# ruanyyyyyyy/point-cloud-process

Hardware: AMD Instinct MI355X
Metric: correspondence-pairs/sec + ms/ICP-iter, 120k-pt KITTI pair (higher is better)
Workload: dtype f64; 1 GPU; point-to-point ICP iteration, 120000 x 120000 KITTI-shaped synthetic scan pair per GPU (BASELINE configs[1]); exact 1-NN via grid; nn=grid, pairs_per_gpu=1, points_src=120000, points_tgt=120000

## Files before the change

include/pcr.h:

```cpp
#ifndef PCR_H
#define PCR_H

#include <stdint.h>

#ifdef __cplusplus
extern "C" {
#endif

#define PCR_API __attribute__((visibility("default")))

enum {
    PCR_OK = 0,
    PCR_E_TOO_FEW_ASSOC = 1,
    PCR_E_INVALID = -1,
    PCR_E_EMPTY = -2,
    PCR_E_NOMEM = -3,
    PCR_E_HIP = -4,
    PCR_E_NO_DEVICE = -5,
    PCR_E_UNSUPPORTED = -6,
    PCR_E_TOO_MANY_ITERS = -7,
    PCR_E_SINGULAR = -8
};

typedef struct pcr_ctx pcr_ctx;
typedef struct pcr_cloud pcr_cloud;
typedef struct pcr_index pcr_index;

PCR_API const char* pcr_strerror(int status);
PCR_API const char* pcr_last_error(const pcr_ctx* ctx);
PCR_API const char* pcr_version(void);

PCR_API int pcr_ctx_create(int device, pcr_ctx** out);
PCR_API int pcr_ctx_destroy(pcr_ctx* ctx);
PCR_API int pcr_ctx_sync(pcr_ctx* ctx);
PCR_API int pcr_ctx_device_info(pcr_ctx* ctx, char* name256, int* cu_count, int64_t* hbm_bytes);

PCR_API int pcr_cloud_upload_f32(pcr_ctx* ctx, const float* xyz, int64_t n, int64_t stride_floats, pcr_cloud** out);
PCR_API int pcr_cloud_upload_f64(pcr_ctx* ctx, const double* xyz, int64_t n, int64_t stride_doubles, pcr_cloud** out);
PCR_API int pcr_cloud_download_f64(pcr_ctx* ctx, const pcr_cloud* cloud, double* xyz_out );
PCR_API int64_t pcr_cloud_size(const pcr_cloud* cloud);
PCR_API int pcr_cloud_reordered(const pcr_cloud* cloud);
PCR_API int pcr_cloud_free(pcr_ctx* ctx, pcr_cloud* cloud);
PCR_API int pcr_cloud_prepare(pcr_ctx* ctx, pcr_cloud* cloud, const pcr_index* index);
PCR_API int pcr_cloud_transform(pcr_ctx* ctx, pcr_cloud* cloud, const double T[16]);

enum { PCR_INDEX_GRID = 0, PCR_INDEX_BRUTE = 1 };
PCR_API int pcr_index_build(pcr_ctx* ctx, const pcr_cloud* target, int kind, double cell, pcr_index** out);
PCR_API int pcr_index_free(pcr_ctx* ctx, pcr_index* index);
PCR_API int pcr_index_kind(const pcr_index* index);
PCR_API double pcr_index_cell(const pcr_index* index);
PCR_API int64_t pcr_index_size(const pcr_index* index);

PCR_API int pcr_nn1(pcr_ctx* ctx, const pcr_index* index, const pcr_cloud* queries, const double* T ,
                    double max_d2, int32_t* idx_out, double* d2_out);

PCR_API int pcr_knn(pcr_ctx* ctx, const pcr_index* index, const double* queries_xyz, int64_t q, int k,
                    int32_t* idx_out, double* dist_out);
PCR_API int pcr_radius(pcr_ctx* ctx, const pcr_index* index, const double* queries_xyz, int64_t q, double radius,
                       int64_t* counts_out, const int64_t* offsets, int32_t* idx_out, double* dist_out);

PCR_API int pcr_radius_small(pcr_ctx* ctx, const pcr_index* index, const double* queries_xyz, int q, double radius, int64_t cap,
                             int64_t* counts_out, int32_t* idx_out, double* dist_out);

enum { PCR_ICP_COMPAT_MAIN = 0,
       PCR_ICP_TOTAL = 1         };
enum { PCR_RMETRIC_FROBENIUS = 0, PCR_RMETRIC_GEODESIC = 1 };
#define PCR_ICP_MAX_LOG 256

typedef struct pcr_icp_params {
    int32_t max_iter;
    double r_thres;
    double t_thres;
    double max_d2;
    int32_t mode;
// ... 328 lines not shown
```

point-cloud-process_amd/_lib.py:

```python
from __future__ import annotations

import ctypes as C
import os
import sys

import numpy as np

_HERE = os.path.dirname(os.path.abspath(__file__))
LIB_PATH = os.environ.get("PCR_LIB_PATH") or os.path.join(_HERE, "libpcr.so")

PCR_OK = 0
PCR_E_TOO_FEW_ASSOC = 1
PCR_E_INVALID = -1
PCR_E_EMPTY = -2
PCR_E_NOMEM = -3
PCR_E_HIP = -4
PCR_E_NO_DEVICE = -5
PCR_E_UNSUPPORTED = -6
PCR_E_TOO_MANY_ITERS = -7
PCR_E_SINGULAR = -8

PCR_INDEX_GRID = 0
PCR_INDEX_BRUTE = 1
PCR_ICP_COMPAT_MAIN = 0
# ... 230 lines not shown
        ("kmeans_converged", C.c_int32),
        ("n_empty", C.c_int32),
        ("n_edges", C.c_int64),
        ("eigenvalues", C.c_double * 8),
        ("residuals", C.c_double * 8),
        ("next_eigenvalue", C.c_double),
        ("inertia", C.c_double),
        ("graph_ms", C.c_double),
        ("solver_ms", C.c_double),
        ("kmeans_ms", C.c_double),
        ("reserved", C.c_double * 4),
    ]


_vp = C.c_void_p
_dp = C.POINTER(C.c_double)
_fp = C.POINTER(C.c_float)
_ip = C.POINTER(C.c_int32)
_lp = C.POINTER(C.c_int64)

SIGNATURES = {
    "pcr_strerror": (C.c_char_p, [C.c_int]),
    "pcr_last_error": (C.c_char_p, [_vp]),
    "pcr_version": (C.c_char_p, []),
    "pcr_ctx_create": (C.c_int, [C.c_int, C.POINTER(_vp)]),
    "pcr_ctx_destroy": (C.c_int, [_vp]),
    "pcr_ctx_sync": (C.c_int, [_vp]),
    "pcr_ctx_device_info": (C.c_int, [_vp, C.c_char_p, C.POINTER(C.c_int), _lp]),
    "pcr_cloud_upload_f32": (C.c_int, [_vp, _fp, C.c_int64, C.c_int64, C.POINTER(_vp)]),
    "pcr_cloud_upload_f64": (C.c_int, [_vp, _dp, C.c_int64, C.c_int64, C.POINTER(_vp)]),
    "pcr_cloud_download_f64": (C.c_int, [_vp, _vp, _dp]),
    "pcr_cloud_size": (C.c_int64, [_vp]),
    "pcr_cloud_reordered": (C.c_int, [_vp]),
    "pcr_cloud_free": (C.c_int, [_vp, _vp]),
    "pcr_cloud_transform": (C.c_int, [_vp, _vp, _dp]),
    "pcr_cloud_prepare": (C.c_int, [_vp, _vp, _vp]),
    "pcr_index_build": (C.c_int, [_vp, _vp, C.c_int, C.c_double, C.POINTER(_vp)]),
    "pcr_index_free": (C.c_int, [_vp, _vp]),
    "pcr_index_kind": (C.c_int, [_vp]),
    "pcr_index_cell": (C.c_double, [_vp]),
    "pcr_index_size": (C.c_int64, [_vp]),
    "pcr_nn1": (C.c_int, [_vp, _vp, _vp, _dp, C.c_double, _ip, _dp]),
    "pcr_knn": (C.c_int, [_vp, _vp, _dp, C.c_int64, C.c_int, _ip, _dp]),
    "pcr_radius": (C.c_int, [_vp, _vp, _dp, C.c_int64, C.c_double, _lp, _lp, _ip, _dp]),
    "pcr_radius_small": (C.c_int, [_vp, _vp, _dp, C.c_int, C.c_double, C.c_int64, _lp, _ip, _dp]),
    "pcr_icp_default_params": (None, [C.POINTER(IcpParams)]),
    "pcr_icp": (C.c_int, [_vp, _vp, _vp, C.POINTER(IcpParams), _dp, C.POINTER(IcpResult)]),
    "pcr_index_set_normals": (C.c_int, [_vp, _vp, _dp]),
    "pcr_index_has_normals": (C.c_int, [_vp]),
    "pcr_icp_plane_default_params": (None, [C.POINTER(IcpPlaneParams)]),
    "pcr_icp_point2plane": (C.c_int, [_vp, _vp, _vp, C.POINTER(IcpPlaneParams), _dp, C.POINTER(IcpPlaneResult)]),
    "pcr_point2plane_moments": (C.c_int, [_vp, _vp, _vp, _dp, C.c_double, _dp]),
    "pcr_point2plane_solve": (C.c_int, [_dp, _dp, _dp, _dp]),
    "pcr_icp_batch": (C.c_int, [C.POINTER(_vp), C.c_int, C.POINTER(Pair), C.c_int64, C.POINTER(IcpParams), C.POINTER(IcpResult), _ip]),
    "pcr_global_default_params": (C.c_int, [C.c_double, C.POINTER(GlobalParams)]),
    "pcr_register_pairs": (C.c_int, [C.POINTER(_vp), C.c_int, C.POINTER(CloudRef), C.c_int64, C.POINTER(PairRef), C.c_int64, C.POINTER(GlobalParams),
                                     C.POINTER(IcpParams), C.POINTER(IcpResult), _ip, _dp]),
    "pcr_match_pairs_fused": (C.c_int, [_vp, _dp, _lp, C.c_int64, _ip, C.c_int64, C.c_int, _ip, _dp, _ip, _dp, _ip, _ip]),
    "pcr_icp_moments": (C.c_int, [_vp, _vp, _vp, _dp, C.c_double, _dp, _dp, _dp]),
    "pcr_procrustes": (C.c_int, [_dp, _dp, C.c_int64, _dp, _dp, _dp]),
    "pcr_homo2tq": (C.c_int, [_dp, _dp]),
    "pcr_voxel_keys": (C.c_int, [_vp, _dp, C.c_int64, C.c_double, _dp, _dp]),
    "pcr_voxel_filter": (C.c_int, [_vp, _dp, C.c_int64, C.c_double, C.c_int, C.c_uint64, _dp, _lp]),
    "pcr_voxel_filter_cloud": (C.c_int, [_vp, _vp, C.c_double, C.c_int, C.c_uint64, C.POINTER(_vp)]),
    "pcr_iss": (C.c_int, [_vp, _vp, C.c_double, C.c_double, C.c_double, C.c_double, C.c_int, _dp, _ip, _ip, C.POINTER(C.c_int)]),
    "pcr_pca": (C.c_int, [_vp, _vp, _dp, _dp, _dp]),
# ... 127 lines not shown
```

point-cloud-process_amd/csrc/pcr_core.hip:

```cpp
#include <algorithm>
#include <cmath>
#include <cstdio>
#include <cstring>
#include <cstdlib>
#include <chrono>
#include <thread>
#include <atomic>
#include <memory>
#include <utility>
#include <vector>
#include "pcr_internal.h"

extern "C" {

const char* pcr_version(void) { return "pcr 0.1 (gfx950, f64)"; }

const char* pcr_strerror(int s) {
    switch (s) {
        case PCR_OK: return "ok";
        case PCR_E_TOO_FEW_ASSOC: return "ICP failed, cannot find enough associations!";
        case PCR_E_INVALID: return "invalid argument";
        case PCR_E_EMPTY: return "empty point cloud";
        case PCR_E_NOMEM: return "out of memory";
        case PCR_E_HIP: return "HIP runtime error";
// ... 543 lines not shown
    hipLaunchKernelGGL(expand_cloud_kernel<S>, dim3(grid), dim3(block), 0, ctx->stream, d_src, (long long)n, (long long)stride, c->d,
                       (unsigned long long*)pcr_counter(ctx, PCR_CW_BOX), h_box_dev);
    PCR_HIP(ctx, hipGetLastError());
    PCR_HIP(ctx, pcr_sync(ctx->stream));
    {
        double lo[3], hi[3];
        bool finite = true;
        for (int k = 0; k < 3; ++k) {
            hi[k] = ordered_value(h_box[k]);
            lo[k] = -ordered_value(h_box[3 + k]);
            finite = finite && std::isfinite(lo[k]) && std::isfinite(hi[k]);
        }
        if (finite) {
            c->has_bbox = true;
            for (int k = 0; k < 3; ++k) { c->lo[k] = lo[k] == 0.0 ? 0.0 : lo[k]; c->hi[k] = hi[k]; }
        }
    }
    if (timing) {
        const auto t_2 = std::chrono::steady_clock::now();
        fprintf(stderr, "upload n=%lld stride=%lld: host copy + box %.1f us, expand kernel + sync %.1f us\n", (long long)n, (long long)stride,
                std::chrono::duration_cast<std::chrono::nanoseconds>(t_1 - t_0).count() / 1e3, std::chrono::duration_cast<std::chrono::nanoseconds>(t_2 - t_1).count() / 1e3);
    }
    *out = c.release();
    return PCR_OK;
}

__global__ void cloud_rows_kernel(const pcr_pt* __restrict__ in, long long n, pcr_pt* __restrict__ out) {
    long long i = (long long)blockIdx.x * blockDim.x + threadIdx.x;
    if (i >= n) return;
    const pcr_pt p = in[i];
    out[p.id] = p;
}

int pcr_cloud_rows(pcr_ctx* ctx, const pcr_cloud* c, pcr_pt* d_out) {
    hipLaunchKernelGGL(cloud_rows_kernel, dim3((unsigned)((c->n + 255) / 256)), dim3(256), 0, ctx->stream, (const pcr_pt*)c->d, (long long)c->n, d_out);
    PCR_HIP(ctx, hipGetLastError());
    return PCR_OK;
}

__global__ void __launch_bounds__(256)
cloud_gather_rows_kernel(const pcr_pt* __restrict__ pts, long long n, const long long* __restrict__ rows, const long long* __restrict__ slot, int m,
                         double* __restrict__ out) {
    const long long i = (long long)blockIdx.x * blockDim.x + threadIdx.x;
    if (i >= n) return;
    const pcr_pt r = pts[i];
    int lo = 0, hi = m;
    while (lo < hi) {
        const int mid = (lo + hi) >> 1;
        if (rows[mid] < r.id) lo = mid + 1; else hi = mid;
    }
    for (; lo < m && rows[lo] == r.id; ++lo) {
        const long long s = slot ? slot[lo] : lo;
        out[3 * s] = r.x; out[3 * s + 1] = r.y; out[3 * s + 2] = r.z;
    }
}

int pcr_cloud_gather_rows(pcr_ctx* ctx, const pcr_cloud* c, const long long* d_rows_sorted, const long long* d_slot, int64_t m, double* d_xyz_out) {
    hipLaunchKernelGGL(cloud_gather_rows_kernel, dim3((unsigned)((c->n + 255) / 256)), dim3(256), 0, ctx->stream, (const pcr_pt*)c->d, (long long)c->n,
                       d_rows_sorted, d_slot, (int)m, d_xyz_out);
    PCR_HIP(ctx, hipGetLastError());
    return PCR_OK;
}

constexpr int64_t PCR_DOWNLOAD_MAX_ROWS = 4096;

extern "C" {
// ... 17 lines not shown
    int grid = (int)((c->n + block - 1) / block);
    hipLaunchKernelGGL(pack_xyz_kernel, dim3(grid), dim3(block), 0, ctx->stream, (const pcr_pt*)c->d, (long long)c->n, d_tmp);
    PCR_HIP(ctx, hipGetLastError());
    PCR_HIP(ctx, hipMemcpyAsync(out, d_tmp, sizeof(double) * 3 * c->n, hipMemcpyDeviceToHost, ctx->stream));
    PCR_HIP(ctx, pcr_sync(ctx->stream));
    return PCR_OK;
}

int pcr_cloud_download_rows(pcr_ctx* ctx, const pcr_cloud* cloud, const int64_t* rows, int64_t m, double* xyz_out) try {
    if (!ctx || !cloud || !rows || !xyz_out || m < 0 || m > PCR_DOWNLOAD_MAX_ROWS) return PCR_E_INVALID;
    if (m == 0) return PCR_OK;
    const int64_t n = cloud->n;
    std::vector<std::pair<long long, long long>> order((size_t)m);
    for (int64_t i = 0; i < m; ++i) {
        if (rows[i] < 0 || rows[i] >= n) return PCR_E_INVALID;
        order[(size_t)i] = {(long long)rows[i], (long long)i};
    }
    std::sort(order.begin(), order.end());
    std::vector<long long> packed(2 * (size_t)m);
    for (int64_t i = 0; i < m; ++i) { packed[(size_t)i] = order[(size_t)i].first; packed[(size_t)(m + i)] = order[(size_t)i].second; }
    hipSetDevice(ctx->device);
    pcr_dev_block d_rows(ctx), d_out(ctx);
    int rc;
    if ((rc = d_rows.alloc(sizeof(long long) * 2 * m)) || (rc = d_out.alloc(sizeof(double) * 3 * m))) return rc;
    PCR_HIP(ctx, hipMemcpyAsync(d_rows.p, packed.data(), sizeof(long long) * 2 * m, hipMemcpyHostToDevice, ctx->stream));
    PCR_HIP(ctx, hipMemsetAsync(d_out.p, 0xff, sizeof(double) * 3 * m, ctx->stream));
    if ((rc = pcr_cloud_gather_rows(ctx, cloud, d_rows.as<long long>(), d_rows.as<long long>() + m, m, d_out.as<double>()))) return rc;
    return pcr_d2h_small(ctx, xyz_out, d_out.p, sizeof(double) * 3 * m);
} PCR_CATCH(ctx)

int64_t pcr_cloud_size(const pcr_cloud* c) { return c ? c->n : 0; }
int pcr_cloud_reordered(const pcr_cloud* c) { return c && c->morton_sorted ? 1 : 0; }

int pcr_cloud_free(pcr_ctx* ctx, pcr_cloud* c) {
    if (!c) return PCR_OK;
    if (!ctx) return PCR_E_INVALID;
    pcr_dev_free(ctx, c->d);
    delete c;
    return PCR_OK;
}

int pcr_cloud_transform(pcr_ctx* ctx, pcr_cloud* c, const double T[16]) {
    if (!ctx || !c || !T) return PCR_E_INVALID;
    hipSetDevice(ctx->device);
    pcr_xform x;
    pcr_xform_from_T(T, &x);
    int block = 256;
    int grid = (int)((c->n + block - 1) / block);
    c->has_bbox = false;
    hipLaunchKernelGGL(transform_cloud_kernel, dim3(grid), dim3(block), 0, ctx->stream, c->d, (long long)c->n, x);
    PCR_HIP(ctx, hipGetLastError());
    return PCR_OK;
}

}
```

point-cloud-process_amd/csrc/pcr_grid.hip:

```cpp
#include <cfloat>
#include <cmath>
#include <cstdio>
#include <cstring>
#include <rocprim/rocprim.hpp>
#include "pcr_internal.h"
#include "pcr_grid_build_dev.h"
#include "pcr_sort.h"

__global__ void bbox_partial_kernel(const pcr_pt* __restrict__ pts, long long n, double* __restrict__ part) {
    __shared__ double s[6][256];
    double mn[3] = {DBL_MAX, DBL_MAX, DBL_MAX}, mx[3] = {-DBL_MAX, -DBL_MAX, -DBL_MAX};
    for (long long i = (long long)blockIdx.x * blockDim.x + threadIdx.x; i < n; i += (long long)gridDim.x * blockDim.x) {
        pcr_pt p = pts[i];
        mn[0] = fmin(mn[0], p.x); mx[0] = fmax(mx[0], p.x);
        mn[1] = fmin(mn[1], p.y); mx[1] = fmax(mx[1], p.y);
        mn[2] = fmin(mn[2], p.z); mx[2] = fmax(mx[2], p.z);
    }
    for (int k = 0; k < 3; ++k) { s[k][threadIdx.x] = mn[k]; s[3 + k][threadIdx.x] = mx[k]; }
    __syncthreads();
    for (int st = 128; st > 0; st >>= 1) {
        if ((int)threadIdx.x < st) {
            for (int k = 0; k < 3; ++k) {
                s[k][threadIdx.x] = fmin(s[k][threadIdx.x], s[k][threadIdx.x + st]);
                s[3 + k][threadIdx.x] = fmax(s[3 + k][threadIdx.x], s[3 + k][threadIdx.x + st]);
            }
        }
        __syncthreads();
    }
    if (threadIdx.x < 6) part[blockIdx.x * 6 + threadIdx.x] = s[threadIdx.x][0];
}

template <typename K>
__device__ static inline unsigned long long full_key(K k) { return (unsigned long long)k | MORTON_BIAS3; }

template <typename K>
__global__ void __launch_bounds__(256)
morton_keys_var_kernel(const pcr_pt* __restrict__ pts, long long n, double lox, double loy, double loz, double inv, unsigned long long mask,
                       K* __restrict__ keys, unsigned int* __restrict__ vals) {
    const long long i = (long long)blockIdx.x * blockDim.x + threadIdx.x;
    if (i >= n) return;
    const pcr_pt p = pts[i];
    keys[i] = (K)(morton_key(p.x, p.y, p.z, lox, loy, loz, inv) & mask);
    vals[i] = (unsigned int)i;
}

template <typename K>
__global__ void __launch_bounds__(256)
gather_count_kernel(const pcr_pt* __restrict__ pts, const unsigned int* __restrict__ perm, const K* __restrict__ keys, long long n, int levels,
                    pcr_pt* __restrict__ out, unsigned int* __restrict__ counts, unsigned int* __restrict__ host_counts) {
    __shared__ unsigned int s_cnt[PCR_MAX_LEVELS];
    __shared__ int s_last;
    const long long i = (long long)blockIdx.x * blockDim.x + threadIdx.x;
    if (levels > 0 && threadIdx.x < PCR_MAX_LEVELS) s_cnt[threadIdx.x] = 0;
    if (i < n) out[i] = pts[perm[i]];
    if (levels <= 0) return;
    __syncthreads();
    const unsigned long long k = i < n ? full_key(keys[i]) : 0ull, kp = (i < n && i > 0) ? full_key(keys[i - 1]) : 0ull;
    count_run_starts(k, kp, (unsigned long long)i, i < n, levels, s_cnt);
    __syncthreads();
    if ((int)threadIdx.x < levels && s_cnt[threadIdx.x])
        __hip_atomic_fetch_add(&counts[threadIdx.x * 64 + (blockIdx.x & 63u)], s_cnt[threadIdx.x], __ATOMIC_RELAXED, __HIP_MEMORY_SCOPE_AGENT);
    asm volatile("s_waitcnt vmcnt(0)" ::: "memory");
    if (threadIdx.x == 0) s_last = __hip_atomic_fetch_add(&counts[PCR_MAX_LEVELS * 64], 1u, __ATOMIC_RELAXED, __HIP_MEMORY_SCOPE_AGENT) == gridDim.x - 1 ? 1 : 0;
    __syncthreads();
    if (!s_last) return;
    for (int l = threadIdx.x >> 6; l < PCR_MAX_LEVELS; l += 4) {
        unsigned int v = __hip_atomic_load(&counts[l * 64 + (threadIdx.x & 63)], __ATOMIC_RELAXED, __HIP_MEMORY_SCOPE_AGENT);
        counts[l * 64 + (threadIdx.x & 63)] = 0;
#pragma unroll
        for (int d = 32; d > 0; d >>= 1) v += __shfl_xor(v, d, 64);
        if ((threadIdx.x & 63) == 0) host_counts[l] = v;
    }
    if (threadIdx.x == 0) counts[PCR_MAX_LEVELS * 64] = 0;
}

// ... 57 lines not shown
        return PCR_OK;
    }
    return pcr_bbox(ctx, c->d, c->n, lo, hi);
}

void pcr_grid_plan(const double lo[3], const double hi[3], long long n, double cell, double* cell_out, int* levels_out) {
    double ext[3] = {hi[0] - lo[0], hi[1] - lo[1], hi[2] - lo[2]};
    double emax = fmax(ext[0], fmax(ext[1], ext[2]));
    if (!(cell > 0)) {
        double e[3] = {ext[0], ext[1], ext[2]};
        if (e[0] < e[1]) std::swap(e[0], e[1]);
        if (e[1] < e[2]) std::swap(e[1], e[2]);
        if (e[0] < e[1]) std::swap(e[0], e[1]);
        double area = e[0] * e[1];
        cell = (area > 0) ? 0.55 * sqrt(area / (double)n) : (emax > 0 ? emax / 64.0 : 1.0);
    }
    double min_cell = emax / 262144.0;
    if (cell < min_cell) cell = min_cell;
    if (!(cell > 0)) cell = 1.0;
    int levels = 1;
    {
        double c = cell;
        while (c < emax * (1.0 + 1e-9) && levels < PCR_MAX_LEVELS) { c *= 4.0; ++levels; }
    }
    *cell_out = cell;
    *levels_out = levels;
}

struct sort_scratch {
    pcr_dev_block keys, keys2, vals, vals2, temp;
    explicit sort_scratch(pcr_ctx* ctx) : keys(ctx), keys2(ctx), vals(ctx), vals2(ctx), temp(ctx) {}
};
template <typename K>
static int morton_sort_records(pcr_ctx* ctx, const pcr_pt* in, long long n, const double lo[3], double inv, int end_bit, int levels, pcr_pt* out,
                               sort_scratch* sc) {
    int rc;
    if ((rc = sc->keys.alloc(sizeof(K) * (size_t)n)) || (rc = sc->keys2.alloc(sizeof(K) * (size_t)n)) || (rc = sc->vals.alloc(sizeof(unsigned int) * n)) ||
        (rc = sc->vals2.alloc(sizeof(unsigned int) * n)))
        return rc;
    K *keys = sc->keys.as<K>(), *keys2 = sc->keys2.as<K>();
    unsigned int *vals = sc->vals.as<unsigned int>(), *vals2 = sc->vals2.as<unsigned int>();
    const int grid_n = (int)((n + 255) / 256);
    const unsigned long long mask = end_bit >= 64 ? ~0ull : (1ull << end_bit) - 1ull;
    hipLaunchKernelGGL(morton_keys_var_kernel<K>, dim3(grid_n), dim3(256), 0, ctx->stream, in, n, lo[0], lo[1], lo[2], inv, mask, keys, vals);
    if ((rc = pcr_sort_pairs_arena(ctx, keys, keys2, vals, vals2, (size_t)n, (unsigned int)end_bit, sc->temp))) return rc;
    unsigned int* h_counts_dev = nullptr;
    if (levels > 0) PCR_HIP(ctx, hipHostGetDevicePointer((void**)&h_counts_dev, ctx->h_pinned, 0));
    hipLaunchKernelGGL(gather_count_kernel<K>, dim3(grid_n), dim3(256), 0, ctx->stream, in, (const unsigned int*)vals2, (const K*)keys2, n, levels, out,
                       ctx->d_cell_counts, h_counts_dev);
    PCR_HIP(ctx, hipGetLastError());
    return PCR_OK;
}

template <typename K>
static int grid_build_tables(pcr_ctx* ctx, pcr_index* idx, const sort_scratch* sc, int levels, const unsigned int* h_counts, const double lo[3], const double hi[3],
                             double cell) {
    const long long n = idx->n;
    int rc;
    pcr_grid_view& v = idx->view;
    memset(&v, 0, sizeof(v));
    v.pts = idx->sorted;
    v.n = n;
    v.levels = levels;
    v.cell0 = cell;
    v.inv_cell0 = 1.0 / cell;
    for (int k = 0; k < 3; ++k) {
        v.lo[k] = lo[k];
        v.origin[k] = 0.5 * (lo[k] + hi[k]);
    }
    size_t cell_slots = 0, block_slots = 0;
    for (int l = 0; l < levels; ++l) {
        const pcr_table_caps c = pcr_table_caps_of(h_counts[l], 16);
        v.mask[l] = c.cap / 4 - 1;
        v.bmask[l] = c.bcap - 1;
        cell_slots += c.cap;
        block_slots += c.bcap;
    }
    idx->cell_pool_bytes = sizeof(pcr_cell_slot) * cell_slots;
// ... 1 lines not shown
    if ((rc = pcr_dev_alloc(ctx, idx->cell_pool_bytes, (void**)&idx->cell_pool)) || (rc = pcr_dev_alloc(ctx, idx->block_pool_bytes, (void**)&idx->block_pool)) ||
        (rc = pcr_dev_alloc(ctx, sizeof(pcr_grid_view), (void**)&idx->d_view)))
        return rc;
    for (size_t l = 0, co = 0, bo = 0; l < (size_t)levels; ++l) {
        v.table[l] = idx->cell_pool + co;
        v.btable[l] = idx->block_pool + bo;
        co += 4 * ((size_t)v.mask[l] + 1);
        bo += (size_t)v.bmask[l] + 1;
    }
    const int grid_n = (int)((n + 255) / 256);
    const unsigned long long words = cell_slots + 2 * block_slots;
    int gi = (int)((words + 256 * 4 - 1) / (256 * 4));
    if (gi > 4 * ctx->cu_count) gi = 4 * ctx->cu_count;
    hipLaunchKernelGGL(init_pools_kernel, dim3(gi < 1 ? 1 : gi), dim3(256), 0, ctx->stream, idx->cell_pool, (unsigned long long)cell_slots, idx->block_pool,
                       (unsigned long long)block_slots);
    hipLaunchKernelGGL(insert_cells_var_kernel<K>, dim3(grid_n), dim3(256), 0, ctx->stream, sc->keys2.as<const K>(), n, idx->view);
    hipLaunchKernelGGL(insert_blocks_var_kernel<K>, dim3(grid_n), dim3(256), 0, ctx->stream, sc->keys2.as<const K>(), n, idx->view, idx->d_view);
    PCR_HIP(ctx, hipGetLastError());
    return PCR_OK;
}

int pcr_grid_build(pcr_ctx* ctx, const pcr_cloud* tgt, double cell, pcr_index* idx) {
    const long long n = tgt->n;
    int rc;
    double lo[3] = {idx->lo[0], idx->lo[1], idx->lo[2]}, hi[3] = {idx->hi[0], idx->hi[1], idx->hi[2]};
    int levels = 1;
    pcr_grid_plan(lo, hi, n, cell, &cell, &levels);
    idx->cell = cell;
    const double inv = 1.0 / cell;
    const int end_bit = pcr_morton_end_bit(lo, hi, inv);
    if ((rc = pcr_dev_alloc(ctx, sizeof(pcr_pt) * n, (void**)&idx->sorted))) return rc;
    sort_scratch sc(ctx);
    const bool k32 = end_bit <= 32;
    rc = k32 ? morton_sort_records<unsigned int>(ctx, tgt->d, n, lo, inv, end_bit, levels, idx->sorted, &sc)
             : morton_sort_records<unsigned long long>(ctx, tgt->d, n, lo, inv, end_bit, levels, idx->sorted, &sc);
    if (rc == PCR_OK && pcr_sync(ctx->stream) != hipSuccess) { ctx->last_error = "hipStreamSynchronize (index build)"; rc = PCR_E_HIP; }
    if (rc == PCR_OK) {
        unsigned int h_counts[PCR_MAX_LEVELS];
        memcpy(h_counts, ctx->h_pinned, sizeof(h_counts));
        rc = k32 ? grid_build_tables<unsigned int>(ctx, idx, &sc, levels, h_counts, lo, hi, cell)
                 : grid_build_tables<unsigned long long>(ctx, idx, &sc, levels, h_counts, lo, hi, cell);
    }
    return rc;
}

int pcr_cloud_morton_sort(pcr_ctx* ctx, pcr_cloud* c, double cell) {
    if (c->morton_sorted || c->n < 2) { c->morton_sorted = true; return PCR_OK; }
    const long long n = c->n;
    double lo[3], hi[3];
    int rc = pcr_cloud_bbox(ctx, c, lo, hi);
    if (rc) return rc;
    const double emax = fmax(hi[0] - lo[0], fmax(hi[1] - lo[1], hi[2] - lo[2]));
    if (!(cell > 0)) cell = emax > 0 ? emax / 1024.0 : 1.0;
    if (cell < emax / 262144.0) cell = emax / 262144.0;
    pcr_dev_block d_out(ctx);
    if ((rc = d_out.alloc(sizeof(pcr_pt) * n))) return rc;
    const int end_bit = pcr_morton_end_bit(lo, hi, 1.0 / cell);
    sort_scratch sc(ctx);
    rc = end_bit <= 32 ? morton_sort_records<unsigned int>(ctx, c->d, n, lo, 1.0 / cell, end_bit, 0, d_out.as<pcr_pt>(), &sc)
                       : morton_sort_records<unsigned long long>(ctx, c->d, n, lo, 1.0 / cell, end_bit, 0, d_out.as<pcr_pt>(), &sc);
    if (rc) return rc;
    pcr_dev_free(ctx, c->d);
    c->d = d_out.release<pcr_pt>();
    c->morton_sorted = true;
    return PCR_OK;
}

void pcr_grid_free(pcr_ctx* ctx, pcr_index* idx) {
    if (idx->d_view) pcr_dev_free(ctx, idx->d_view);
    idx->d_view = nullptr;
    if (idx->sorted) pcr_dev_free(ctx, idx->sorted);
    idx->sorted = nullptr;
    if (idx->cell_pool) pcr_dev_free(ctx, idx->cell_pool);
    if (idx->block_pool) pcr_dev_free(ctx, idx->block_pool);
    idx->cell_pool = nullptr;
    idx->block_pool = nullptr;
}
```

point-cloud-process_amd/csrc/pcr_grid_search.hip:

```cpp
#include <atomic>
#include <chrono>
#include <cmath>
#include <cstdlib>
#include <cstring>
#include "pcr_descent.h"
#include "pcr_icp_step.h"

constexpr unsigned int HARD_SCAN_T = 192;
constexpr int HARD_STACK = 160;
constexpr long long ID_NONE = 0x7fffffffffffffffll;
constexpr int H_NLIST = 32;
constexpr int H_CSTRIDE = 32;
__host__ __device__ static inline unsigned int hard_list_cap(long long nq) {
    const long long halves = (nq + 15) / 16;
    return (unsigned int)(((halves + H_NLIST - 1) / H_NLIST) * 16 + 64);
}

template <int G>
__device__ static inline void group_best(double& bd2, long long& bid, unsigned int& bpos) {
#pragma unroll
    for (int off = G / 2; off > 0; off >>= 1) {
        const double od2 = __shfl_xor(bd2, off, 64);
        const long long oid = __shfl_xor(bid, off, 64);
        const unsigned int opos = __shfl_xor(bpos, off, 64);
// ... 1599 lines not shown
    block_state_from_T0(st, T0.v);
    if (plog && threadIdx.x == 0) plog[3 * PCR_ICP_MAX_LOG] = (unsigned int)__builtin_amdgcn_s_memrealtime();
}

bool pcr_pass_fixed_scale(const double lo[3], const double hi[3], long long nq, double max_d2, double* scale, double* inv_scale, double* lin) {
    double r2 = 0.0;
    for (int k = 0; k < 3; ++k) r2 += 0.25 * (hi[k] - lo[k]) * (hi[k] - lo[k]);
    const double R = sqrt(r2) + sqrt(max_d2);
    const double M = (double)nq * fmax(fmax(R * R, max_d2), 1.0);
    int ex = 0;
    frexp(M, &ex);
    int exq = 0;
    frexp(M / (double)nq, &exq);
    const int F = (61 - ex < 51 - exq) ? 61 - ex : 51 - exq;
    if (!(M > 0) || !std::isfinite(M) || F < 20) return false;
    *scale = ldexp(1.0, F);
    *inv_scale = ldexp(1.0, -F);
    int ex1 = 0, exq1 = 0;
    frexp((double)nq * fmax(R, 1.0), &ex1);
    frexp(fmax(R, 1.0), &exq1);
    const int F1 = (61 - ex1 < 51 - exq1) ? 61 - ex1 : 51 - exq1;
    const double e = ldexp(1.0, -(F + 1)) / sqrt(3.0 * (double)nq);
    *lin = (e > 1e-11 && F1 > F) ? ldexp(1.0, F1 - F) : 1.0;
    return true;
}

static std::atomic<int> g_loops_in_flight[64];
struct loop_guard {
    std::atomic<int>& n;
    explicit loop_guard(int device) : n(g_loops_in_flight[(unsigned int)device % 64u]) { n.fetch_add(1); }
    ~loop_guard() { n.fetch_sub(1); }
};

int pcr_grid_icp_loop(pcr_ctx* ctx, const pcr_index* idx, pcr_cloud* qc, const pcr_icp_params* params, const double T0[16],
                      pcr_icp_result* res) {
    const loop_guard in_flight(ctx->device);
    const auto h_t0 = std::chrono::steady_clock::now();
    auto h_us = [&](std::chrono::steady_clock::time_point a) { return std::chrono::duration_cast<std::chrono::nanoseconds>(std::chrono::steady_clock::now() - a).count() / 1e3; };
    for (double& v : ctx->pass_host_us) v = 0.0;
    const char* const wait_s = getenv("PCR_PASS_INLINE");
    const int wait_env = wait_s ? atoi(wait_s) : -1;
    const bool gated = (params->max_d2 > 0) && std::isfinite(params->max_d2);
    int rc = pcr_cloud_morton_sort(ctx, qc, idx->cell);
    if (rc) return rc;
    const int64_t nq = qc->n;
    int grid = (int)((nq + 1023) / 1024);
    if (grid > ctx->cu_count) grid = ctx->cu_count;
    double sc_f = 0, sc_i = 0, sc_lin = 1.0;
    const bool fused = gated && nq <= PASS_MAX_NQ && getenv("PCR_ICP_NO_FUSED") == nullptr &&
                       pcr_pass_fixed_scale(idx->lo, idx->hi, nq, params->max_d2, &sc_f, &sc_i, &sc_lin);
    grid_scratch sc(ctx);
    pcr_dev_block st_blk(ctx);
    if ((rc = grid_scratch_alloc(&sc, nq, false, !fused)) || (rc = sc.prev_xyz.alloc(24 * (size_t)nq))) return rc;
    const char* const lb_s = getenv("PCR_PASS_GATE_LB");
    const bool gate_bounds = !(lb_s && atoi(lb_s) == 0);
    const pass_layout pl = pass_scratch_layout(nq, 1, true, gate_bounds);
    pass_args pa{};
    if (fused) {
        if ((rc = sc.acc.alloc(8 * pl.zero_words)) || (rc = sc.tile_cost.alloc(sizeof(unsigned int) * 4 * (size_t)wtile_blocks(nq))) ||
            (rc = sc.items.alloc(8 * pl.item_words)))
            return rc;
        pa.cap = pl.cap;
        pa.items = sc.items.as<unsigned long long>();
        pa.tile_cost = sc.tile_cost.as<unsigned int>();
        pa.acc = sc.acc.as<unsigned long long>();
        pa.sync = pa.acc + pl.sync_word;
        pa.plog = (unsigned int*)(pa.acc + pl.log_word);
        pa.prev_xyz = sc.prev_xyz.as<wt_xyz>();
        if (gate_bounds) {
            pa.gate_est = pa.acc + pl.est_word;
            pa.gate_lb = pa.acc + pl.lb_word;
        }
        pa.scale = sc_f;
        pa.inv_scale = sc_i;
        pa.lin = sc_lin;
        pa.inv_lin = 1.0 / sc_lin;
    }
    if ((rc = pcr_ensure_scratch(ctx, sizeof(double) * PCR_NMOM * (size_t)grid)) || (rc = st_blk.alloc(sizeof(pcr_icp_dev_state)))) return rc;
    pcr_icp_dev_state* const d_st = st_blk.as<pcr_icp_dev_state>();
    static_assert(sizeof(pcr_icp_dev_state) <= 8192, "state must fit the pinned staging buffer");
    pcr_icp_dev_state* h_st = (pcr_icp_dev_state*)ctx->h_state;
    memset(h_st, 0, sizeof(*h_st));
    pcr::icp_state_from_T0(T0, h_st);
// ... 253 lines not shown
```

point-cloud-process_amd/csrc/pcr_icp.hip:

```cpp
#include <cmath>
#include <cstdio>
#include <cstring>
#include <cstdlib>
#include <atomic>
#include <chrono>
#include <thread>
#include <vector>
#include "pcr_internal.h"
#include "pcr_linalg.h"
#include "pcr_icp_step.h"

extern "C" {

int pcr_index_build(pcr_ctx* ctx, const pcr_cloud* target, int kind, double cell, pcr_index** out) try {
    if (!ctx || !target || !out) return PCR_E_INVALID;
    *out = nullptr;
    if (target->n <= 0) return PCR_E_EMPTY;
    if (kind != PCR_INDEX_GRID && kind != PCR_INDEX_BRUTE) return PCR_E_INVALID;
    hipSetDevice(ctx->device);
    pcr_index_guard idx(ctx, new pcr_index());
    idx->kind = kind;
    idx->n = target->n;
    memset(&idx->view, 0, sizeof(idx->view));
    int rc = pcr_cloud_bbox(ctx, target, idx->lo, idx->hi);
// ... 87 lines not shown
    memcpy(res->T, compat ? T_cur : st->T_total, sizeof(T_cur));
    return PCR_OK;
}

extern "C" {

int pcr_icp_moments(pcr_ctx* ctx, const pcr_cloud* source, const pcr_index* index, const double* T, double max_d2,
                    double moments_out[18], double origin_out[3], double* sum_d2_out) try {
    if (!ctx || !source || !index || !moments_out) return PCR_E_INVALID;
    hipSetDevice(ctx->device);
    pcr_xform x;
    pcr_xform_from_T(T, &x);
    pcr_dev_block d_mom(ctx);
    int rc = d_mom.alloc(sizeof(double) * PCR_NMOM);
    if (rc) return rc;
    if ((rc = icp_pass(ctx, index, const_cast<pcr_cloud*>(source), &x, max_d2, 0, d_mom.as<double>()))) return rc;
    PCR_HIP(ctx, hipMemcpyAsync(ctx->h_pinned, d_mom.p, sizeof(double) * PCR_NMOM, hipMemcpyDeviceToHost, ctx->stream));
    PCR_HIP(ctx, pcr_sync(ctx->stream));
    memcpy(moments_out, ctx->h_pinned, sizeof(double) * 18);
    if (sum_d2_out) *sum_d2_out = ctx->h_pinned[18];
    if (origin_out)
        for (int k = 0; k < 3; ++k) origin_out[k] = index->view.origin[k];
    return PCR_OK;
} PCR_CATCH(ctx)

int pcr_icp(pcr_ctx* ctx, pcr_cloud* source, const pcr_index* index, const pcr_icp_params* params, const double T0[16],
            pcr_icp_result* res) try {
    if (!ctx || !source || !index || !params || !T0 || !res) return PCR_E_INVALID;
    if (params->max_iter > PCR_ICP_MAX_LOG) return PCR_E_TOO_MANY_ITERS;
    if (source->n <= 0) return PCR_E_EMPTY;
    hipSetDevice(ctx->device);
    memset(res, 0, sizeof(*res));
    if (index->kind == PCR_INDEX_GRID) {
        const int rs = pcr_cloud_morton_sort(ctx, source, index->cell);
        if (rs) return rs;
    }
    source->has_bbox = false;
    PCR_HIP(ctx, hipEventRecord(ctx->ev0, ctx->stream));
    int rc;
    if (index->kind == PCR_INDEX_GRID) {
        if ((rc = pcr_grid_icp_loop(ctx, index, source, params, T0, res))) return rc;
    } else {
        pcr_icp_dev_state st;
        memset(&st, 0, sizeof(st));
        pcr::icp_state_from_T0(T0, &st);
        const pcr_icp_loop_args la = pcr_icp_loop_args_from(params);
        double nn_ms = 0;
        for (int it = 0; it < params->max_iter && !st.stop; ++it) {
            if (ctx->profile) PCR_HIP(ctx, hipEventRecord(ctx->ev2, ctx->stream));
            rc = pcr_brute_icp_pass(ctx, index, source->d, source->n, &st.x, params->max_d2, 1, ctx->h_pinned);
            if (rc) return rc;
            if (ctx->profile) PCR_HIP(ctx, hipEventRecord(ctx->ev3, ctx->stream));
            PCR_HIP(ctx, pcr_sync(ctx->stream));
            float ms = 0;
            if (ctx->profile) hipEventElapsedTime(&ms, ctx->ev2, ctx->ev3);
            nn_ms += ms;
            pcr::icp_step(&st, ctx->h_pinned, index->view.origin, la, st.r_diff, st.t_diff);
        }
        if ((rc = pcr_icp_finish(ctx, source, params, &st, res))) return rc;
        res->nn_kernel_ms = nn_ms;
    }
    if (index->kind == PCR_INDEX_GRID && ctx->loop_dev_ms > 0.0) {
        res->device_ms = ctx->loop_dev_ms;
        return res->status;
    }
    PCR_HIP(ctx, hipEventRecord(ctx->ev1, ctx->stream));
    PCR_HIP(ctx, pcr_event_sync(ctx->ev1));
// ... 56 lines not shown
```

point-cloud-process_amd/csrc/pcr_internal.h:

```cpp
#pragma once
#include <hip/hip_runtime.h>
#include <stdint.h>
#include <exception>
#include <new>
#include <string>
#include <vector>
#include "pcr.h"

#define PCR_HIDDEN __attribute__((visibility("hidden")))

struct __attribute__((aligned(32))) pcr_pt {
    double x, y, z;
    long long id;
};

struct pcr_xform {
    double r[9];
    double t[3];
};

constexpr int PCR_MAX_LEVELS = 12;
constexpr int PCR_COORD_BITS = 21;
constexpr long long PCR_COORD_BIAS = 1ll << 20;
constexpr long long PCR_COORD_MAX = (1ll << PCR_COORD_BITS) - 1;
// ... 191 lines not shown
    {16, 14},
    {48, 2},
    {64, 1},
    {72, 1},
    {80, 1},
    {88, 1},
    {96, 1},
    {112, 1},
    {116, 1},
    {117, 2},
    {120, 2},
    {124, 1},
    {125, 3},
    {136, 1},
};
constexpr bool pcr_cw_disjoint() {
    int end = 0;
    for (int u = 0; u < PCR_CW_USERS; ++u) {
        if (PCR_CW_SPAN[u].words < 1 || PCR_CW_SPAN[u].first < end) return false;
        end = PCR_CW_SPAN[u].first + PCR_CW_SPAN[u].words;
    }
    return end <= PCR_HARD_COUNTERS;
}
static_assert(pcr_cw_disjoint(), "d_counters: two users share a word, or a user has no row");
static inline unsigned int* pcr_counter(const pcr_ctx* ctx, pcr_cw user, int k = 0) { return ctx->d_counters + PCR_CW_SPAN[user].first + k; }
PCR_HIDDEN int pcr_ensure_scratch(pcr_ctx* ctx, size_t partial_bytes);
PCR_HIDDEN void pcr_xform_from_T(const double* T, pcr_xform* x);
PCR_HIDDEN void pcr_prof_mark(pcr_ctx* ctx, int k);
PCR_HIDDEN void pcr_prof_finish(pcr_ctx* ctx);

PCR_HIDDEN int pcr_bbox(pcr_ctx* ctx, const pcr_pt* pts, long long n, double lo[3], double hi[3]);
PCR_HIDDEN int pcr_cloud_bbox(pcr_ctx* ctx, const pcr_cloud* c, double lo[3], double hi[3]);
PCR_HIDDEN int pcr_grid_build(pcr_ctx* ctx, const pcr_cloud* tgt, double cell, pcr_index* idx);
PCR_HIDDEN int pcr_cloud_morton_sort(pcr_ctx* ctx, pcr_cloud* c, double cell);
PCR_HIDDEN void pcr_grid_free(pcr_ctx* ctx, pcr_index* idx);
PCR_HIDDEN int pcr_grid_nn1(pcr_ctx* ctx, const pcr_index* idx, pcr_cloud* qc, const pcr_xform* x, double max_d2, int32_t* d_idx,
                            double* d_d2);
PCR_HIDDEN int pcr_grid_icp_pass(pcr_ctx* ctx, const pcr_index* idx, pcr_cloud* qc, const pcr_xform* x, double max_d2,
                                 int write_back, double* d_moments);
PCR_HIDDEN int pcr_brute_build(pcr_ctx* ctx, const pcr_cloud* tgt, pcr_index* idx);
PCR_HIDDEN void pcr_brute_free(pcr_ctx* ctx, pcr_index* idx);
PCR_HIDDEN int pcr_brute_nn1(pcr_ctx* ctx, const pcr_index* idx, const pcr_pt* q, int64_t nq, const pcr_xform* x,
                             double max_d2, int32_t* d_idx, double* d_d2);
PCR_HIDDEN int pcr_brute_last_fallback(pcr_ctx* ctx, unsigned int* out);
PCR_HIDDEN int pcr_brute_icp_pass(pcr_ctx* ctx, const pcr_index* idx, pcr_pt* q, int64_t nq, const pcr_xform* x,
                                  double max_d2, int write_back, double* d_moments);

PCR_HIDDEN void pcr_point2plane_free(pcr_ctx* ctx, pcr_index* idx);

constexpr int PCR_NMOM = 20;

struct __attribute__((aligned(16))) pcr_icp_dev_state {
    pcr_xform x;
    double T_total[16];
    double R_last[9], t_last[3];
    double V[9];
    double cost, mean_d2;
    long long n_assoc;
    int it;
    int stop;
    int converged;
    int status;
    int first;
    int passes;
    double r_diff[PCR_ICP_MAX_LOG], t_diff[PCR_ICP_MAX_LOG];
};
struct pcr_icp_loop_args {
// ... 52 lines not shown
```

point-cloud-process_amd/device.py:

```python
from __future__ import annotations

import ctypes as C
import threading

import numpy as np

from . import _lib as L

_default_ctx = {}
_lock = threading.Lock()


class Context:

    def __init__(self, device=0, shared=False):
        self._h = C.c_void_p()
        self.device = int(device)
        L.check(L.lib().pcr_ctx_create(self.device, C.byref(self._h)))
        if shared:
            self.set_shared(True)

    def set_shared(self, shared=True):
        L.check(L.lib().pcr_ctx_set_shared(self.handle, 1 if shared else 0), self.handle)

# ... 88 lines not shown
        self.n = int(n)

    @classmethod
    def upload(cls, points, ctx=None):
        ctx = ctx or default_context()
        arr = points_of(points)
        h = C.c_void_p()
        if arr.shape[0] == 0:
            raise L.PcrError(L.PCR_E_EMPTY)
        if arr.dtype == np.float32:
            a = np.ascontiguousarray(arr)
            st = L.lib().pcr_cloud_upload_f32(ctx.handle, a.ctypes.data_as(C.POINTER(C.c_float)), a.shape[0], a.shape[1], C.byref(h))
        else:
            a = np.ascontiguousarray(arr, dtype=np.float64)
            st = L.lib().pcr_cloud_upload_f64(ctx.handle, L.dptr(a), a.shape[0], a.shape[1], C.byref(h))
        L.check(st, ctx.handle)
        return cls(ctx, h, arr.shape[0])

    @property
    def handle(self):
        if not self._h:
            raise RuntimeError("cloud freed")
        return self._h

    def download(self):
        out = np.empty((self.n, 3), dtype=np.float64)
        L.check(L.lib().pcr_cloud_download_f64(self.ctx.handle, self.handle, L.dptr(out)), self.ctx.handle)
        return out

    def download_rows(self, rows):
        rows = np.ascontiguousarray(rows, dtype=np.int64).reshape(-1)
        out = np.empty((len(rows), 3), dtype=np.float64)
        L.check(L.lib().pcr_cloud_download_rows(self.ctx.handle, self.handle, L.lptr(rows), len(rows), L.dptr(out)), self.ctx.handle)
        return out

    def transform(self, T):
        T = L.as_f64(T).reshape(16)
        L.check(L.lib().pcr_cloud_transform(self.ctx.handle, self.handle, L.dptr(T)), self.ctx.handle)
        return self

    def prepare(self, index):
        L.check(L.lib().pcr_cloud_prepare(self.ctx.handle, self.handle, index.handle), self.ctx.handle)
        return self

    def free(self):
        if self._h:
            L.lib().pcr_cloud_free(self.ctx.handle, self._h)
            self._h = C.c_void_p()

    def __len__(self):
        return self.n

    def __del__(self):
        try:
            self.free()
        except Exception:
            pass


class TargetIndex:

    KINDS = {"grid": L.PCR_INDEX_GRID, "brute": L.PCR_INDEX_BRUTE}

    def __init__(self, target, kind="grid", cell=0.0, ctx=None):
        ctx = ctx or (target.ctx if isinstance(target, DeviceCloud) else default_context())
        self.ctx = ctx
# ... 187 lines not shown
```

Before: 3.369 billion correspondences/s.

## Order query points along a Hilbert curve for the fused ICP pass

When the fused ICP pass applies, source points are now sorted along a 3D Hilbert curve, or a 2D Hilbert curve with a minor third axis for flat scans, instead of Morton order. The target index keeps Morton order. The aim is better spatial locality between neighbouring threads, so grid-cell lookups and cache use are more coherent across a wavefront. Hilbert key computation is costlier, and the sort may use more bits. A new API also exposes the reordered row ids.

```diff
diff --git a/include/pcr.h b/include/pcr.h
--- a/include/pcr.h
+++ b/include/pcr.h
@@ -40,6 +40,7 @@
 PCR_API int pcr_cloud_download_f64(pcr_ctx* ctx, const pcr_cloud* cloud, double* xyz_out );
 PCR_API int64_t pcr_cloud_size(const pcr_cloud* cloud);
 PCR_API int pcr_cloud_reordered(const pcr_cloud* cloud);
+PCR_API int pcr_cloud_order(pcr_ctx* ctx, const pcr_cloud* cloud, int64_t* rows_out );
 PCR_API int pcr_cloud_free(pcr_ctx* ctx, pcr_cloud* cloud);
 PCR_API int pcr_cloud_prepare(pcr_ctx* ctx, pcr_cloud* cloud, const pcr_index* index);
 PCR_API int pcr_cloud_transform(pcr_ctx* ctx, pcr_cloud* cloud, const double T[16]);
diff --git a/point-cloud-process_amd/_lib.py b/point-cloud-process_amd/_lib.py
--- a/point-cloud-process_amd/_lib.py
+++ b/point-cloud-process_amd/_lib.py
@@ -286,6 +286,7 @@
     "pcr_cloud_download_f64": (C.c_int, [_vp, _vp, _dp]),
     "pcr_cloud_size": (C.c_int64, [_vp]),
     "pcr_cloud_reordered": (C.c_int, [_vp]),
+    "pcr_cloud_order": (C.c_int, [_vp, _vp, _lp]),
     "pcr_cloud_free": (C.c_int, [_vp, _vp]),
     "pcr_cloud_transform": (C.c_int, [_vp, _vp, _dp]),
     "pcr_cloud_prepare": (C.c_int, [_vp, _vp, _vp]),
diff --git a/point-cloud-process_amd/csrc/pcr_core.hip b/point-cloud-process_amd/csrc/pcr_core.hip
--- a/point-cloud-process_amd/csrc/pcr_core.hip
+++ b/point-cloud-process_amd/csrc/pcr_core.hip
@@ -599,6 +599,11 @@
     out[p.id] = p;
 }
 
+__global__ void cloud_ids_kernel(const pcr_pt* __restrict__ in, long long n, long long* __restrict__ out) {
+    long long i = (long long)blockIdx.x * blockDim.x + threadIdx.x;
+    if (i < n) out[i] = in[i].id;
+}
+
 int pcr_cloud_rows(pcr_ctx* ctx, const pcr_cloud* c, pcr_pt* d_out) {
     hipLaunchKernelGGL(cloud_rows_kernel, dim3((unsigned)((c->n + 255) / 256)), dim3(256), 0, ctx->stream, (const pcr_pt*)c->d, (long long)c->n, d_out);
     PCR_HIP(ctx, hipGetLastError());
@@ -682,6 +687,20 @@
 int64_t pcr_cloud_size(const pcr_cloud* c) { return c ? c->n : 0; }
 int pcr_cloud_reordered(const pcr_cloud* c) { return c && c->morton_sorted ? 1 : 0; }
 
+int pcr_cloud_order(pcr_ctx* ctx, const pcr_cloud* c, int64_t* rows_out) try {
+    if (!ctx || !c || !rows_out) return PCR_E_INVALID;
+    if (c->n <= 0) return PCR_E_EMPTY;
+    hipSetDevice(ctx->device);
+    pcr_dev_block b_ids(ctx);
+    int rc = b_ids.alloc(sizeof(long long) * c->n);
+    if (rc != PCR_OK) return rc;
+    hipLaunchKernelGGL(cloud_ids_kernel, dim3((unsigned)((c->n + 255) / 256)), dim3(256), 0, ctx->stream, (const pcr_pt*)c->d, (long long)c->n, b_ids.as<long long>());
+    PCR_HIP(ctx, hipGetLastError());
+    PCR_HIP(ctx, hipMemcpyAsync(rows_out, b_ids.p, sizeof(long long) * c->n, hipMemcpyDeviceToHost, ctx->stream));
+    PCR_HIP(ctx, pcr_sync(ctx->stream));
+    return PCR_OK;
+} PCR_CATCH(ctx)
+
 int pcr_cloud_free(pcr_ctx* ctx, pcr_cloud* c) {
     if (!c) return PCR_OK;
     if (!ctx) return PCR_E_INVALID;
diff --git a/point-cloud-process_amd/csrc/pcr_curve.h b/point-cloud-process_amd/csrc/pcr_curve.h
--- /dev/null
+++ b/point-cloud-process_amd/csrc/pcr_curve.h
@@ -0,0 +1,88 @@
+#pragma once
+#include "pcr_grid_dev.h"
+
+enum { PCR_CURVE_MORTON = 0, PCR_CURVE_HILBERT3 = 1, PCR_CURVE_HILBERT2_MINOR = 2 };
+
+struct pcr_curve {
+    int mode;
+    int nb;
+    int ax[3];
+    int nb_minor;
+    int bits;
+};
+
+template <int N>
+__host__ __device__ static inline unsigned long long hilbert_index(unsigned int (&X)[N], int nb) {
+    const unsigned int M = 1u << (nb - 1);
+    for (unsigned int Q = M; Q > 1; Q >>= 1) {
+        const unsigned int P = Q - 1;
+#pragma unroll
+        for (int i = 0; i < N; ++i) {
+            if (X[i] & Q) X[0] ^= P;
+            else { const unsigned int t = (X[0] ^ X[i]) & P; X[0] ^= t; X[i] ^= t; }
+        }
+    }
+#pragma unroll
+    for (int i = 1; i < N; ++i) X[i] ^= X[i - 1];
+    unsigned int t = 0;
+    for (unsigned int Q = M; Q > 1; Q >>= 1)
+        if (X[N - 1] & Q) t ^= Q - 1;
+    unsigned long long key = 0;
+#pragma unroll
+    for (int i = 0; i < N; ++i) {
+        const unsigned long long x = X[i] ^ t;
+        for (int b = 0; b < nb; ++b) key |= ((x >> b) & 1ull) << (N * b + (N - 1 - i));
+    }
+    return key;
+}
+
+__host__ __device__ static inline unsigned long long hilbert3_of_cell(unsigned int cx, unsigned int cy, unsigned int cz, int nb) {
+    const unsigned int m = (1u << nb) - 1u;
+    unsigned int X[3] = {cx & m, cy & m, cz & m};
+    return hilbert_index<3>(X, nb);
+}
+
+__host__ __device__ static inline unsigned long long hilbert2_minor_of_cell(unsigned int ca, unsigned int cb, unsigned int cminor, int nb, int nb_minor) {
+    const unsigned int m = (1u << nb) - 1u;
+    unsigned int X[2] = {ca & m, cb & m};
+    return (hilbert_index<2>(X, nb) << nb_minor) | (unsigned long long)(cminor & ((1u << nb_minor) - 1u));
+}
+
+__device__ static inline unsigned long long hilbert3_key(double x, double y, double z, double lox, double loy, double loz, double inv, int nb) {
+    bool clamped = false;
+    const unsigned int cx = (unsigned int)cell_coord(x, lox, inv, &clamped);
+    const unsigned int cy = (unsigned int)cell_coord(y, loy, inv, &clamped);
+    const unsigned int cz = (unsigned int)cell_coord(z, loz, inv, &clamped);
+    return hilbert3_of_cell(cx, cy, cz, nb);
+}
+
+__device__ static inline unsigned long long hilbert2_minor_key(double x, double y, double z, double lox, double loy, double loz, double inv,
+                                                               const pcr_curve& cv) {
+    bool clamped = false;
+    const unsigned int c[3] = {(unsigned int)cell_coord(x, lox, inv, &clamped), (unsigned int)cell_coord(y, loy, inv, &clamped),
+                               (unsigned int)cell_coord(z, loz, inv, &clamped)};
+    const unsigned int ca = cv.ax[0] == 0 ? c[0] : cv.ax[0] == 1 ? c[1] : c[2];
+    const unsigned int cb = cv.ax[1] == 0 ? c[0] : cv.ax[1] == 1 ? c[1] : c[2];
+    const unsigned int cm = cv.ax[2] == 0 ? c[0] : cv.ax[2] == 1 ? c[1] : c[2];
+    return hilbert2_minor_of_cell(ca, cb, cm, cv.nb, cv.nb_minor);
+}
+
+static inline pcr_curve pcr_curve_pick(const double lo[3], const double hi[3], double inv, int end_bit, bool morton) {
+    pcr_curve cv = {PCR_CURVE_MORTON, end_bit / 3, {0, 1, 2}, 0, end_bit};
+    if (morton) return cv;
+    const double e[3] = {hi[0] - lo[0], hi[1] - lo[1], hi[2] - lo[2]};
+    for (int i = 1; i < 3; ++i)
+        for (int j = i; j > 0 && e[cv.ax[j]] > e[cv.ax[j - 1]]; --j) { const int t = cv.ax[j]; cv.ax[j] = cv.ax[j - 1]; cv.ax[j - 1] = t; }
+    if (e[cv.ax[2]] <= 0.25 * e[cv.ax[1]]) {
+        const double kmax = floor(e[cv.ax[2]] * inv) + 2.0;
+        int nbm = 1;
+        while (nbm < cv.nb && (double)(1ll << nbm) <= kmax) ++nbm;
+        cv.mode = PCR_CURVE_HILBERT2_MINOR;
+        cv.nb_minor = nbm;
+        cv.bits = 2 * cv.nb + nbm;
+    } else {
+        cv.mode = PCR_CURVE_HILBERT3;
+        cv.bits = 3 * cv.nb;
+    }
+    return cv;
+}
diff --git a/point-cloud-process_amd/csrc/pcr_grid.hip b/point-cloud-process_amd/csrc/pcr_grid.hip
--- a/point-cloud-process_amd/csrc/pcr_grid.hip
+++ b/point-cloud-process_amd/csrc/pcr_grid.hip
@@ -1,10 +1,12 @@
 #include <cfloat>
 #include <cmath>
 #include <cstdio>
+#include <cstdlib>
 #include <cstring>
 #include <rocprim/rocprim.hpp>
 #include "pcr_internal.h"
 #include "pcr_grid_build_dev.h"
+#include "pcr_curve.h"
 #include "pcr_sort.h"
 
 __global__ void bbox_partial_kernel(const pcr_pt* __restrict__ pts, long long n, double* __restrict__ part) {
@@ -36,11 +38,13 @@
 template <typename K>
 __global__ void __launch_bounds__(256)
 morton_keys_var_kernel(const pcr_pt* __restrict__ pts, long long n, double lox, double loy, double loz, double inv, unsigned long long mask,
-                       K* __restrict__ keys, unsigned int* __restrict__ vals) {
+                       pcr_curve cv, K* __restrict__ keys, unsigned int* __restrict__ vals) {
     const long long i = (long long)blockIdx.x * blockDim.x + threadIdx.x;
     if (i >= n) return;
     const pcr_pt p = pts[i];
-    keys[i] = (K)(morton_key(p.x, p.y, p.z, lox, loy, loz, inv) & mask);
+    keys[i] = cv.mode == PCR_CURVE_HILBERT3         ? (K)hilbert3_key(p.x, p.y, p.z, lox, loy, loz, inv, cv.nb)
+              : cv.mode == PCR_CURVE_HILBERT2_MINOR ? (K)hilbert2_minor_key(p.x, p.y, p.z, lox, loy, loz, inv, cv)
+                                                    : (K)(morton_key(p.x, p.y, p.z, lox, loy, loz, inv) & mask);
     vals[i] = (unsigned int)i;
 }
 
@@ -164,8 +168,8 @@
     explicit sort_scratch(pcr_ctx* ctx) : keys(ctx), keys2(ctx), vals(ctx), vals2(ctx), temp(ctx) {}
 };
 template <typename K>
-static int morton_sort_records(pcr_ctx* ctx, const pcr_pt* in, long long n, const double lo[3], double inv, int end_bit, int levels, pcr_pt* out,
-                               sort_scratch* sc) {
+static int morton_sort_records(pcr_ctx* ctx, const pcr_pt* in, long long n, const double lo[3], double inv, int end_bit, const pcr_curve& cv, int levels,
+                               pcr_pt* out, sort_scratch* sc) {
     int rc;
     if ((rc = sc->keys.alloc(sizeof(K) * (size_t)n)) || (rc = sc->keys2.alloc(sizeof(K) * (size_t)n)) || (rc = sc->vals.alloc(sizeof(unsigned int) * n)) ||
         (rc = sc->vals2.alloc(sizeof(unsigned int) * n)))
@@ -174,8 +178,8 @@
     unsigned int *vals = sc->vals.as<unsigned int>(), *vals2 = sc->vals2.as<unsigned int>();
     const int grid_n = (int)((n + 255) / 256);
     const unsigned long long mask = end_bit >= 64 ? ~0ull : (1ull << end_bit) - 1ull;
-    hipLaunchKernelGGL(morton_keys_var_kernel<K>, dim3(grid_n), dim3(256), 0, ctx->stream, in, n, lo[0], lo[1], lo[2], inv, mask, keys, vals);
-    if ((rc = pcr_sort_pairs_arena(ctx, keys, keys2, vals, vals2, (size_t)n, (unsigned int)end_bit, sc->temp))) return rc;
+    hipLaunchKernelGGL(morton_keys_var_kernel<K>, dim3(grid_n), dim3(256), 0, ctx->stream, in, n, lo[0], lo[1], lo[2], inv, mask, cv, keys, vals);
+    if ((rc = pcr_sort_pairs_arena(ctx, keys, keys2, vals, vals2, (size_t)n, (unsigned int)cv.bits, sc->temp))) return rc;
     unsigned int* h_counts_dev = nullptr;
     if (levels > 0) PCR_HIP(ctx, hipHostGetDevicePointer((void**)&h_counts_dev, ctx->h_pinned, 0));
     hipLaunchKernelGGL(gather_count_kernel<K>, dim3(grid_n), dim3(256), 0, ctx->stream, in, (const unsigned int*)vals2, (const K*)keys2, n, levels, out,
@@ -243,8 +247,9 @@
     if ((rc = pcr_dev_alloc(ctx, sizeof(pcr_pt) * n, (void**)&idx->sorted))) return rc;
     sort_scratch sc(ctx);
     const bool k32 = end_bit <= 32;
-    rc = k32 ? morton_sort_records<unsigned int>(ctx, tgt->d, n, lo, inv, end_bit, levels, idx->sorted, &sc)
-             : morton_sort_records<unsigned long long>(ctx, tgt->d, n, lo, inv, end_bit, levels, idx->sorted, &sc);
+    const pcr_curve cv = pcr_curve_pick(lo, hi, inv, end_bit, true);
+    rc = k32 ? morton_sort_records<unsigned int>(ctx, tgt->d, n, lo, inv, end_bit, cv, levels, idx->sorted, &sc)
+             : morton_sort_records<unsigned long long>(ctx, tgt->d, n, lo, inv, end_bit, cv, levels, idx->sorted, &sc);
     if (rc == PCR_OK && pcr_sync(ctx->stream) != hipSuccess) { ctx->last_error = "hipStreamSynchronize (index build)"; rc = PCR_E_HIP; }
     if (rc == PCR_OK) {
         unsigned int h_counts[PCR_MAX_LEVELS];
@@ -255,7 +260,7 @@
     return rc;
 }
 
-int pcr_cloud_morton_sort(pcr_ctx* ctx, pcr_cloud* c, double cell) {
+int pcr_cloud_morton_sort(pcr_ctx* ctx, pcr_cloud* c, double cell, bool keep_morton) {
     if (c->morton_sorted || c->n < 2) { c->morton_sorted = true; return PCR_OK; }
     const long long n = c->n;
     double lo[3], hi[3];
@@ -267,9 +272,11 @@
     pcr_dev_block d_out(ctx);
     if ((rc = d_out.alloc(sizeof(pcr_pt) * n))) return rc;
     const int end_bit = pcr_morton_end_bit(lo, hi, 1.0 / cell);
+    const char* const curve_s = getenv("PCR_QUERY_CURVE");
+    const pcr_curve cv = pcr_curve_pick(lo, hi, 1.0 / cell, end_bit, keep_morton || (curve_s && strcmp(curve_s, "morton") == 0));
     sort_scratch sc(ctx);
-    rc = end_bit <= 32 ? morton_sort_records<unsigned int>(ctx, c->d, n, lo, 1.0 / cell, end_bit, 0, d_out.as<pcr_pt>(), &sc)
-                       : morton_sort_records<unsigned long long>(ctx, c->d, n, lo, 1.0 / cell, end_bit, 0, d_out.as<pcr_pt>(), &sc);
+    rc = end_bit <= 32 ? morton_sort_records<unsigned int>(ctx, c->d, n, lo, 1.0 / cell, end_bit, cv, 0, d_out.as<pcr_pt>(), &sc)
+                       : morton_sort_records<unsigned long long>(ctx, c->d, n, lo, 1.0 / cell, end_bit, cv, 0, d_out.as<pcr_pt>(), &sc);
     if (rc) return rc;
     pcr_dev_free(ctx, c->d);
     c->d = d_out.release<pcr_pt>();
diff --git a/point-cloud-process_amd/csrc/pcr_grid_search.hip b/point-cloud-process_amd/csrc/pcr_grid_search.hip
--- a/point-cloud-process_amd/csrc/pcr_grid_search.hip
+++ b/point-cloud-process_amd/csrc/pcr_grid_search.hip
@@ -1655,6 +1655,17 @@
     ~loop_guard() { n.fetch_sub(1); }
 };
 
+bool pcr_grid_pass_fused(const pcr_index* idx, int64_t nq, const pcr_icp_params* params, double* scale, double* inv_scale, double* lin) {
+    double sc_f = 0, sc_i = 0, sc_lin = 1.0;
+    const bool gated = (params->max_d2 > 0) && std::isfinite(params->max_d2);
+    const bool fused = gated && nq <= PASS_MAX_NQ && getenv("PCR_ICP_NO_FUSED") == nullptr &&
+                       pcr_pass_fixed_scale(idx->lo, idx->hi, nq, params->max_d2, &sc_f, &sc_i, &sc_lin);
+    if (scale) *scale = sc_f;
+    if (inv_scale) *inv_scale = sc_i;
+    if (lin) *lin = sc_lin;
+    return fused;
+}
+
 int pcr_grid_icp_loop(pcr_ctx* ctx, const pcr_index* idx, pcr_cloud* qc, const pcr_icp_params* params, const double T0[16],
                       pcr_icp_result* res) {
     const loop_guard in_flight(ctx->device);
@@ -1664,14 +1675,13 @@
     const char* const wait_s = getenv("PCR_PASS_INLINE");
     const int wait_env = wait_s ? atoi(wait_s) : -1;
     const bool gated = (params->max_d2 > 0) && std::isfinite(params->max_d2);
-    int rc = pcr_cloud_morton_sort(ctx, qc, idx->cell);
-    if (rc) return rc;
     const int64_t nq = qc->n;
     int grid = (int)((nq + 1023) / 1024);
     if (grid > ctx->cu_count) grid = ctx->cu_count;
     double sc_f = 0, sc_i = 0, sc_lin = 1.0;
-    const bool fused = gated && nq <= PASS_MAX_NQ && getenv("PCR_ICP_NO_FUSED") == nullptr &&
-                       pcr_pass_fixed_scale(idx->lo, idx->hi, nq, params->max_d2, &sc_f, &sc_i, &sc_lin);
+    const bool fused = pcr_grid_pass_fused(idx, nq, params, &sc_f, &sc_i, &sc_lin);
+    int rc = pcr_cloud_morton_sort(ctx, qc, idx->cell, !fused);
+    if (rc) return rc;
     grid_scratch sc(ctx);
     pcr_dev_block st_blk(ctx);
     if ((rc = grid_scratch_alloc(&sc, nq, false, !fused)) || (rc = sc.prev_xyz.alloc(24 * (size_t)nq))) return rc;
diff --git a/point-cloud-process_amd/csrc/pcr_icp.hip b/point-cloud-process_amd/csrc/pcr_icp.hip
--- a/point-cloud-process_amd/csrc/pcr_icp.hip
+++ b/point-cloud-process_amd/csrc/pcr_icp.hip
@@ -143,7 +143,7 @@
     hipSetDevice(ctx->device);
     memset(res, 0, sizeof(*res));
     if (index->kind == PCR_INDEX_GRID) {
-        const int rs = pcr_cloud_morton_sort(ctx, source, index->cell);
+        const int rs = pcr_cloud_morton_sort(ctx, source, index->cell, !pcr_grid_pass_fused(index, source->n, params));
         if (rs) return rs;
     }
     source->has_bbox = false;
diff --git a/point-cloud-process_amd/csrc/pcr_internal.h b/point-cloud-process_amd/csrc/pcr_internal.h
--- a/point-cloud-process_amd/csrc/pcr_internal.h
+++ b/point-cloud-process_amd/csrc/pcr_internal.h
@@ -247,7 +247,9 @@
 PCR_HIDDEN int pcr_bbox(pcr_ctx* ctx, const pcr_pt* pts, long long n, double lo[3], double hi[3]);
 PCR_HIDDEN int pcr_cloud_bbox(pcr_ctx* ctx, const pcr_cloud* c, double lo[3], double hi[3]);
 PCR_HIDDEN int pcr_grid_build(pcr_ctx* ctx, const pcr_cloud* tgt, double cell, pcr_index* idx);
-PCR_HIDDEN int pcr_cloud_morton_sort(pcr_ctx* ctx, pcr_cloud* c, double cell);
+PCR_HIDDEN int pcr_cloud_morton_sort(pcr_ctx* ctx, pcr_cloud* c, double cell, bool keep_morton = false);
+PCR_HIDDEN bool pcr_grid_pass_fused(const pcr_index* idx, int64_t nq, const pcr_icp_params* params, double* scale = nullptr, double* inv_scale = nullptr,
+                                    double* lin = nullptr);
 PCR_HIDDEN void pcr_grid_free(pcr_ctx* ctx, pcr_index* idx);
 PCR_HIDDEN int pcr_grid_nn1(pcr_ctx* ctx, const pcr_index* idx, pcr_cloud* qc, const pcr_xform* x, double max_d2, int32_t* d_idx,
                             double* d_d2);
diff --git a/point-cloud-process_amd/device.py b/point-cloud-process_amd/device.py
--- a/point-cloud-process_amd/device.py
+++ b/point-cloud-process_amd/device.py
@@ -144,6 +144,11 @@
         rows = np.ascontiguousarray(rows, dtype=np.int64).reshape(-1)
         out = np.empty((len(rows), 3), dtype=np.float64)
         L.check(L.lib().pcr_cloud_download_rows(self.ctx.handle, self.handle, L.lptr(rows), len(rows), L.dptr(out)), self.ctx.handle)
+        return out
+
+    def order(self):
+        out = np.empty(self.n, dtype=np.int64)
+        L.check(L.lib().pcr_cloud_order(self.ctx.handle, self.handle, L.lptr(out)), self.ctx.handle)
         return out
 
     def transform(self, T):
```

Result: faster. 3.470 billion correspondences/s, median of 6 (+3.0%).
